# IntptrMax/YoloSharp

Hardware: NVIDIA H100
Metric: images/sec YOLOv8n 3x640x640 (higher is better)
Workload: dtype f16

## Files before the change

yolosharp_b200/csrc/conv_tc.cu:

```cuda
#include <cuda.h>

#include <algorithm>
#include <cstdio>
#include <cstdlib>
#include <cstring>
#include <map>
#include <vector>

#include "common.cuh"
#include "tc_ptx.cuh"

namespace yb {

typedef CUresult (*EncodeTiledFn)(CUtensorMap*, CUtensorMapDataType, cuuint32_t, void*, const cuuint64_t*,
                                  const cuuint64_t*, const cuuint32_t*, const cuuint32_t*, CUtensorMapInterleave,
                                  CUtensorMapSwizzle, CUtensorMapL2promotion, CUtensorMapFloatOOBfill);
static EncodeTiledFn get_encode_fn(std::string* err);

enum TcMode { TC_TAP = 0, TC_HALO = 1, TC_S2P = 2 };

struct TcArgs {
  CUtensorMap tmA;
  const uint8_t* wpk;
  __half* out;
  const __half* res;
  const float* bias;
  int out_pitch, out_coff, res_pitch, res_coff;
  int Ho, Wo;
  int imgs;
  int tiles_w, tiles_h;
  int BW, BH;
  int n_tile, n_tiles;
  int ksz, stride, pad;
  int Cin, BK, chunks;
  int act;
  int mode;
  int stages_a, stages_b;
  uint32_t a_bytes, b_bytes;
  uint32_t a_stride, b_stride;
  uint32_t sbo_a, sbo_b;
  uint32_t row_bytes;
  uint32_t layout_a, layout_b;
  int total_tiles;
  int b_resident;
  int ksteps;
  int epi_mode, dA, dCtot, da0, dch0, dWl, dHW;
  float dstride;
  float* pred;
  uint64_t m_ntiles, m_tpi, m_tw, m_bw;
  int* done_ctr;
  const int* dep_ctr;
  int dep_expect;
  uint64_t m_ohw;
  int* tile_ctr;
  int tile_batch;
  long long* dbg;
  const uint8_t* w2;
  const float* bias2;
  uint32_t w2_off, w2_bytes, b2_stride, sbo_b2, layout_b2;
  int BK2, n2, act1;
};

struct TcConvPlan {
  TcArgs args;
  ConvParams p;
  bool flat;
  int occ;
  bool small;
  size_t smem;
  int grid;
  uint8_t* wpk = nullptr;
  void (*kernel)(TcArgs) = nullptr;
  int fold16 = 0;
};

__device__ __forceinline__ int fdiv(int x, uint64_t magic) { return (int)(((uint64_t)(uint32_t)x * magic) >> 40); }

__device__ __forceinline__ float silu_fast(float v) { return __fdividef(v, 1.0f + __expf(-v)); }
__device__ __forceinline__ float silu_tanh(float v) {
  const float h = 0.5f * v;
  float t;
  asm("tanh.approx.f32 %0, %1;" : "=f"(t) : "f"(h));
  return fmaf(h, t, h);
}

__device__ __forceinline__ uint32_t pack_h2(float x, float y) {
  const __half2 h = __floats2half2_rn(x, y);
  return *reinterpret_cast<const uint32_t*>(&h);
}

constexpr int TC_CONSUMERS = 256;
constexpr int TC_THREADS = TC_CONSUMERS + 32;
constexpr int TC_CONSUMER_WARPS = TC_CONSUMERS / 32;
constexpr int TC_MAX_COUT = 1024;
constexpr int TC_MAX_STAGES = 12;
constexpr int HALO_BW = 8, HALO_BH = 16;

constexpr int TQ = 32;
__device__ __forceinline__ void tq_publish(int* s_tile, volatile int* s_head, int li, int tile) {
  s_tile[li & (TQ - 1)] = tile;
  __threadfence_block();
  *s_head = li + 1;
}
__device__ __forceinline__ int tq_get(const int* s_tile, const volatile int* s_head, int li) {
  const long long t0 = clock64();
  while (*s_head <= li)
    if (clock64() - t0 > 4000000000ll) __trap();
  __threadfence_block();
  return reinterpret_cast<const volatile int*>(s_tile)[li & (TQ - 1)];
}
struct TileDraw {
  int tile, nxt, left, batch, total;
  int* ctr;
  __device__ __forceinline__ TileDraw(int* c, int b, int tot)
      : tile((int)blockIdx.x), nxt(tot), left(1), batch(b), total(tot), ctr(c) {
    if (ctr && tile < total) nxt = (int)gridDim.x + atomicAdd(ctr, batch);
  }
  __device__ __forceinline__ void advance() {
    if (!ctr) { tile += gridDim.x; return; }
    if (--left > 0) { tile++; return; }
    tile = nxt;
    left = batch;
    if (tile < total) nxt = (int)gridDim.x + atomicAdd(ctr, batch);
  }
};

__device__ __forceinline__ void dep_wait_image(const int* ctr, int img, int expect) {
  const long long t0 = clock64();
  while (true) {
    int v;
    asm volatile("ld.acquire.gpu.global.s32 %0, [%1];" : "=r"(v) : "l"(ctr + img) : "memory");
    if (v >= expect) break;
    __nanosleep(100);
    if (clock64() - t0 > 4000000000ll) __trap();
  }
}

template <int NT16, int KK>
__device__ __forceinline__ void tc_mainloop(const TcArgs& a, float* acc, int wg, uint32_t smemA, uint32_t smemB, uint32_t fullA,
                                            uint32_t emptyA, uint32_t fullB, uint32_t emptyB, int& sa, uint32_t& pa, int& sb,
                                            uint32_t& pb) {
  const bool resident = a.b_resident != 0, halo = a.mode != TC_TAP, s2p = a.mode == TC_S2P;
  const uint32_t a_hi = wg_desc_hi(a.sbo_a, a.layout_a), b_hi = wg_desc_hi(a.sbo_b, a.layout_b);
  const uint32_t a_stride16 = a.a_stride >> 4, b_stride16 = a.b_stride >> 4;
  const uint32_t a_lo0 = wg_desc_lo(smemA) + (uint32_t)wg * 8 * a.sbo_a;
  const uint32_t b_lo0 = wg_desc_lo(smemB);
  constexpr uint32_t ROW16 = KK * 2;
  const int ra = a.stages_a, rb = a.stages_b;
  const bool leader = (threadIdx.x & 31) == 0;
  uint32_t pend0 = 0, pend1 = 0;
  uint32_t scale = 0;
  auto step = [&](uint32_t a_lo, uint32_t b_lo, uint32_t relA, uint32_t relB) {
    wg_fence();
#pragma unroll
    for (int k = 0; k < KK; k++) {
      wg_mma_n<NT16, false>(acc, a_lo + 2 * k, a_hi, b_lo + 2 * k, b_hi, ROW16, scale);
      scale = 1;
    }
    wg_commit();
    wg_wait<1>();
    __syncwarp();
    if (leader) {
      if (pend0) mbar_arrive(pend0);
      if (pend1) mbar_arrive(pend1);
    }
    pend0 = relA;
    pend1 = relB;
  };
  if (halo) {
    for (int ch = 0; ch < a.chunks; ch++) {
      mbar_wait(fullA + 8 * sa, pa);
      const uint32_t a_lo = a_lo0 + sa * a_stride16;
      const uint32_t slotA = emptyA + 8 * sa;
      if (++sa == ra) { sa = 0; pa ^= 1; }
#pragma unroll
      for (int t = 0; t < 9; t++) {
        const uint32_t TAP_HALO = (uint32_t)((t / 3) * (HALO_BW + 2) + (t % 3)) * ROW16;
        const uint32_t TAP_S2P = (uint32_t)((t / 3) * (HALO_BW + 1) + (t % 3 != 0 ? 1 : 0)) * 2 * ROW16 +
                                 (t % 3 != 1 ? ROW16 : 0);
// ... 252 lines not shown
      if (a.b_resident)
        for (int ks = 0; ks < a.ksteps; ks++)
          bulk_load_1d(smemB + ks * a.b_stride, a.wpk + (size_t)ks * a.b_stride, a.b_bytes, bfull);
      if (N2_16 > 0) bulk_load_1d(smem0 + a.w2_off, a.w2, a.w2_bytes, bfull);
    }
  }
  if (a.dep_ctr == nullptr) asm volatile("griddepcontrol.wait;" ::: "memory");

  const bool dyn = a.tile_ctr != nullptr;
  if (warp == TC_CONSUMER_WARPS) {
    if (lane == 0) {
      const int ra = a.stages_a, rb = a.b_resident ? 0 : a.stages_b;
      int sa = 0, sb = 0;
      uint32_t pa = 0, pb = 0;
      int li = 0;
      TileDraw td(a.tile_ctr, a.tile_batch, a.total_tiles);
      int dep_ready = -1;
      for (; td.tile < a.total_tiles; li++) {
        const int tile = td.tile;
        if (a.dep_ctr != nullptr) {
          const int mt0 = fdiv(tile, a.m_ntiles);
          int i0, i1;
          if (a.imgs == 1 && a.Ho == 1) {
            const int p0 = mt0 * 128, p1 = min(p0 + 127, a.Wo - 1);
            i0 = fdiv(p0, a.m_ohw); i1 = fdiv(p1, a.m_ohw);
          } else {
            i0 = i1 = fdiv(mt0, a.m_tpi);
          }
          if (i1 != dep_ready || i0 != i1) {
            for (int im = i0; im <= i1; im++)
              if (im != dep_ready) dep_wait_image(a.dep_ctr, im, a.dep_expect);
            dep_ready = i1;
            asm volatile("fence.proxy.async.global;" ::: "memory");
          }
        }
        if (dyn) tq_publish(s_tile, &s_head, li, tile);
        const int mt = fdiv(tile, a.m_ntiles);
        const int nt = tile - mt * a.n_tiles;
        const int img = fdiv(mt, a.m_tpi);
        const int r = mt - img * tiles_per_img;
        const int th = fdiv(r, a.m_tw), tw = r - th * a.tiles_w;
        const int wbase = tw * a.BW * a.stride - a.pad;
        const int hbase = th * a.BH * a.stride - a.pad;
        auto load_b = [&](int t, int ch) {
          mbar_wait(emptyB + 8 * sb, pb ^ 1);
          mbar_arrive_expect_tx(fullB + 8 * sb, a.b_bytes);
          bulk_load_1d(smemB + sb * a.b_stride, a.wpk + (size_t)((nt * taps + t) * a.chunks + ch) * a.b_stride, a.b_bytes,
                       fullB + 8 * sb);
          if (++sb == rb) { sb = 0; pb ^= 1; }
        };
        if (a.mode != TC_TAP) {
          for (int ch = 0; ch < a.chunks; ch++) {
            mbar_wait(emptyA + 8 * sa, pa ^ 1);
            mbar_arrive_expect_tx(fullA + 8 * sa, a.a_bytes);
            tma_load_4d(smemA + sa * a.a_stride, &a.tmA, fullA + 8 * sa, ch * a.BK, a.mode == TC_S2P ? tw * a.BW - 1 : wbase,
                        hbase, img);
            if (++sa == ra) { sa = 0; pa ^= 1; }
            if (!a.b_resident)
              for (int t = 0; t < taps; t++) load_b(t, ch);
          }
        } else {
          for (int t = 0; t < taps; t++) {
            const int kh = a.ksz == 3 ? (t >= 6 ? 2 : (t >= 3 ? 1 : 0)) : 0, kw = t - kh * a.ksz;
            for (int ch = 0; ch < a.chunks; ch++) {
              mbar_wait(emptyA + 8 * sa, pa ^ 1);
              mbar_arrive_expect_tx(fullA + 8 * sa, a.a_bytes);
              tma_load_4d(smemA + sa * a.a_stride, &a.tmA, fullA + 8 * sa, ch * a.BK, wbase + kw, hbase + kh, img);
              if (++sa == ra) { sa = 0; pa ^= 1; }
              if (!a.b_resident) load_b(t, ch);
            }
          }
        }
        td.advance();
      }
      if (dyn) tq_publish(s_tile, &s_head, li, -1);
    }
  } else {
    const int wg = warp >> 2;
    int sa = 0, sb = 0;
    uint32_t pa = 0, pb = 0;
    if (a.b_resident || N2_16 > 0) mbar_wait(bfull, 0);
    int pend_img = -1, pend_cnt = 0;
    const bool dbg_on = a.dbg && blockIdx.x == 0 && threadIdx.x == 0;
    for (int li = 0;; li++) {
      const int tile = dyn ? tq_get(s_tile, &s_head, li) : (int)blockIdx.x + li * (int)gridDim.x;
      if (tile < 0 || tile >= a.total_tiles) break;
      if (dbg_on && li < 16) a.dbg[li * 8 + 0] = clock64();
      float acc[NT16 * 8];
      switch (a.BK) {
        case 64: tc_mainloop<NT16, 4>(a, acc, wg, smemA, smemB, fullA, emptyA, fullB, emptyB, sa, pa, sb, pb); break;
        case 32: tc_mainloop<NT16, 2>(a, acc, wg, smemA, smemB, fullA, emptyA, fullB, emptyB, sa, pa, sb, pb); break;
        default: tc_mainloop<NT16, 1>(a, acc, wg, smemA, smemB, fullA, emptyA, fullB, emptyB, sa, pa, sb, pb); break;
      }
      if (dbg_on && li < 16) a.dbg[li * 8 + 3] = clock64();
      const int mt = fdiv(tile, a.m_ntiles);
      const int nt = tile - mt * a.n_tiles;
      const int img = fdiv(mt, a.m_tpi);
      const int r = mt - img * tiles_per_img;
      const int th = fdiv(r, a.m_tw), tw = r - th * a.tiles_w;
      const int n0 = nt * a.n_tile;
      if constexpr (N2_16 > 0) {
        switch (a.BK2) {
          case 64: tc_fold<NT16, N2_16, 4>(a, acc, s_bias, s_bias + TC_FOLD_BIAS, smem0 + a.w2_off, img, th, tw, wg); break;
          case 32: tc_fold<NT16, N2_16, 2>(a, acc, s_bias, s_bias + TC_FOLD_BIAS, smem0 + a.w2_off, img, th, tw, wg); break;
          default: tc_fold<NT16, N2_16, 1>(a, acc, s_bias, s_bias + TC_FOLD_BIAS, smem0 + a.w2_off, img, th, tw, wg); break;
        }
        if (dbg_on && li < 16) a.dbg[li * 8 + 6] = clock64();
        continue;
      }
      bool valid[2];
      int wo[2];
      tc_epilogue<NT16>(a, acc, s_bias + n0, n0, img, th, tw, wg, valid, wo);
      if (a.done_ctr != nullptr && a.epi_mode == EPI_STORE) {
        const bool flat1 = a.imgs == 1 && a.Ho == 1;
        const int im[2] = {flat1 ? fdiv(min(wo[0], a.Wo - 1), a.m_ohw) : img, flat1 ? fdiv(min(wo[1], a.Wo - 1), a.m_ohw) : img};
        chain_count(a, valid, im, pend_img, pend_cnt);
      }
      if (dbg_on && li < 16) a.dbg[li * 8 + 6] = clock64();
    }
    if (pend_img >= 0) {
      __threadfence();
      __syncwarp();
      if (lane == 0) atomicAdd(a.done_ctr + pend_img, pend_cnt);
    }
  }
}

__global__ void pack_weights_kernel(const __half* __restrict__ w, uint8_t* __restrict__ out, int n_tile, int n_tiles,
                                    int taps, int chunks, int BK, int Cin, uint32_t b_stride, long long pieces) {
  const long long i = (long long)blockIdx.x * blockDim.x + threadIdx.x;
  if (i >= pieces) return;
  const int c16 = BK / 8;
  const int c = (int)(i % c16);
  long long q = i / c16;
  const int r = (int)(q % n_tile); q /= n_tile;
  const int ch = (int)(q % chunks); q /= chunks;
  const int t = (int)(q % taps);
  const int nt = (int)(q / taps);
  const size_t K = (size_t)taps * Cin;
  if (ch * BK + c * 8 >= Cin) return;
  const int4 v = *reinterpret_cast<const int4*>(w + (size_t)(nt * n_tile + r) * K + (size_t)t * Cin + ch * BK + c * 8);
  const int sw = BK == 64 ? (r & 7) : (BK == 32 ? ((r >> 1) & 3) : ((r >> 2) & 1));
  uint8_t* slab = out + (size_t)((nt * taps + t) * chunks + ch) * b_stride;
  *reinterpret_cast<int4*>(slab + (size_t)r * BK * 2 + ((c ^ sw) << 4)) = v;
}

static EncodeTiledFn get_encode_fn(std::string* err) {
  static EncodeTiledFn fn = nullptr;
  if (fn) return fn;
  void* p = nullptr;
  cudaDriverEntryPointQueryResult qres;
  cudaError_t e = cudaGetDriverEntryPoint("cuTensorMapEncodeTiled", &p, cudaEnableDefault, &qres);
  if (e != cudaSuccess || qres != cudaDriverEntryPointSuccess || !p) {
    if (err) *err = "cuTensorMapEncodeTiled entry point not found";
    cudaGetLastError();
    return nullptr;
  }
  fn = (EncodeTiledFn)p;
  return fn;
}

bool tc_conv_supported(const ConvParams& p) {
  if (p.Cin % 16 || p.Cout % 16 || p.Cout > TC_MAX_COUT) return false;
  if (!((p.k == 1 && p.stride == 1) || (p.k == 3 && (p.stride == 1 || p.stride == 2)))) return false;
  if (p.in.coff % 8 || p.in.pitch % 8 || p.out.coff % 8 || p.out.pitch % 8) return false;
  if (p.res.base && (p.res.coff % 8 || p.res.pitch % 8)) return false;
  return true;
}

static int plan_small() {
  const char* v = getenv("YB_PLAN_SMALL");
  return v ? atoi(v) : 0;
}

static int pick_n_tile(int cout) {
  const int cap = plan_small() ? 128 : 256;
  if (cout <= cap) return cout;
  int best = 16;
  for (int n = 16; n <= cap; n += 16)
    if (cout % n == 0) best = n;
  return best;
}

static int tc_num_sms() {
  static int num_sms = 0;
  if (!num_sms) {
    int dev = 0;
    cudaGetDevice(&dev);
    cudaDeviceGetAttribute(&num_sms, cudaDevAttrMultiProcessorCount, dev);
  }
  return num_sms;
}

static bool tc_size_rings(TcConvPlan* plan, size_t extra, int max_occ) {
  TcArgs& a = plan->args;
  const ConvParams& p = plan->p;
  const int num_sms = tc_num_sms();
  const size_t b_all = (size_t)a.ksteps * a.b_stride;
  const int m_tiles = plan->flat ? (p.B * p.Ho * p.Wo + 127) / 128
                                 : p.B * ((p.Wo + a.BW - 1) / a.BW) * ((p.Ho + a.BH - 1) / a.BH);
  const size_t full = 200 * 1024 > extra ? 200 * 1024 - extra : 0;
  plan->occ = 1;
  a.stages_a = 0;
  for (int occ = 2; occ >= 1; occ--) {
    const size_t budget = occ == 2 ? (104 * 1024 > extra ? 104 * 1024 - extra : 0) : full;
    const bool small = m_tiles * a.n_tiles <= 2 * num_sms;
    if (occ == 2 && (a.n_tile > 64 || max_occ < 2)) continue;
    a.b_resident = (a.n_tiles == 1 && b_all + 3 * (size_t)a.a_stride <= budget) ? 1 : 0;
    if (occ == 2 && !plan_small() && !small && !a.b_resident && a.n_tiles == 1 && b_all + 3 * (size_t)a.a_stride <= full) continue;
    if (a.b_resident) {
      a.stages_a = (int)std::min<size_t>(a.mode != TC_TAP ? (a.chunks > 1 ? 8 : 6) : TC_MAX_STAGES, (budget - b_all) / a.a_stride);
      a.stages_b = 0;
    } else if (a.mode != TC_TAP) {
      a.stages_a = (int)std::min<size_t>(3, std::max<size_t>(2, (budget / 3) / a.a_stride));
      const size_t rest = budget > (size_t)a.stages_a * a.a_stride ? budget - (size_t)a.stages_a * a.a_stride : 0;
      a.stages_b = (int)std::min<size_t>(TC_MAX_STAGES, rest / a.b_stride);
    } else {
      a.stages_a = a.stages_b = (int)std::min<size_t>(8, budget / (a.a_stride + a.b_stride));
    }
    const size_t rings = (size_t)a.stages_a * a.a_stride + (a.b_resident ? b_all : (size_t)a.stages_b * a.b_stride);
    a.w2_off = (uint32_t)rings;
    plan->smem = rings + extra + 1024;
    const bool fits = a.stages_a >= 2 && (a.b_resident || a.stages_b >= ((occ == 2 && a.mode != TC_TAP) ? 3 : 2)) && rings <= budget;
    if (fits && (occ == 1 || small || a.stages_a >= 3 || plan_small())) { plan->occ = occ; break; }
    if (occ == 1) a.stages_a = 0;
  }
  plan->small = m_tiles * a.n_tiles <= 2 * num_sms;
  plan->grid = num_sms * plan->occ;
  if (plan_small() && plan->occ == 2) plan->grid = num_sms;
  return !(a.stages_a < 2 || (!a.b_resident && a.stages_b < 2));
}

TcConvPlan* tc_conv_plan_create(const ConvParams& p, std::string* err) {
  EncodeTiledFn encode = get_encode_fn(err);
  if (!encode) return nullptr;
  TcConvPlan* plan = new TcConvPlan();
  plan->p = p;
  TcArgs& a = plan->args;
  memset(&a, 0, sizeof(a));
  a.out = reinterpret_cast<__half*>(p.out.base);
  a.res = reinterpret_cast<const __half*>(p.res.base);
  a.bias = p.bias;
  a.out_pitch = p.out.pitch; a.out_coff = p.out.coff;
  a.res_pitch = p.res.pitch; a.res_coff = p.res.coff;
  a.ksz = p.k; a.stride = p.stride; a.pad = p.pad;
  a.Cin = p.Cin;
  const bool s2p_ok = p.k == 3 && p.stride == 2 && p.in.coff == 0 && p.in.pitch == p.Cin && p.Cin <= 32 && p.in.W % 2 == 0;
  a.mode = (p.k == 3 && p.stride == 1) ? TC_HALO : (s2p_ok ? TC_S2P : TC_TAP);
  auto padded = [&](int bk) { return (p.Cin + bk - 1) / bk * bk; };
  a.BK = padded(64) * 100 <= p.Cin * 135 ? 64 : (padded(32) * 100 <= p.Cin * 135 ? 32 : 16);
  a.chunks = (p.Cin + a.BK - 1) / a.BK;
  a.act = p.act;
  a.n_tile = pick_n_tile(p.Cout);
  a.n_tiles = p.Cout / a.n_tile;
  const CUtensorMapSwizzle swz = a.BK == 64 ? CU_TENSOR_MAP_SWIZZLE_128B
                                            : (a.BK == 32 ? CU_TENSOR_MAP_SWIZZLE_64B : CU_TENSOR_MAP_SWIZZLE_32B);
  a.layout_a = a.layout_b = a.BK == 64 ? 1 : (a.BK == 32 ? 2 : 3);
  a.row_bytes = a.BK * 2;
  a.sbo_a = a.sbo_b = (8 * a.row_bytes) >> 4;
  CUtensorMapSwizzle swz_a = swz;
  if (a.mode == TC_S2P) {
    swz_a = a.BK == 32 ? CU_TENSOR_MAP_SWIZZLE_128B : CU_TENSOR_MAP_SWIZZLE_64B;
    a.layout_a = a.BK == 32 ? 1 : 2;
  }

  plan->flat = (p.k == 1 && p.stride == 1);
  const size_t esz = 2;
  cuuint64_t gdim[4], gstr[3];
  cuuint32_t box[4], estr[4];
  char* base = reinterpret_cast<char*>(p.in.base) + (size_t)p.in.coff * esz;
  if (plan->flat) {
    const cuuint64_t npix = (cuuint64_t)p.B * p.in.H * p.in.W;
    gdim[0] = p.Cin; gdim[1] = npix; gdim[2] = 1; gdim[3] = 1;
    gstr[0] = (cuuint64_t)p.in.pitch * esz; gstr[1] = gstr[0] * npix; gstr[2] = gstr[1];
    a.BW = 128; a.BH = 1;
    box[0] = a.BK; box[1] = 128; box[2] = 1; box[3] = 1;
    estr[0] = estr[1] = estr[2] = estr[3] = 1;
  } else {
    gdim[0] = p.Cin; gdim[1] = p.in.W; gdim[2] = p.in.H; gdim[3] = p.B;
    gstr[0] = (cuuint64_t)p.in.pitch * esz;
    gstr[1] = gstr[0] * p.in.W;
    gstr[2] = gstr[1] * p.in.H;
    if (a.mode == TC_HALO) {
      a.BW = HALO_BW; a.BH = HALO_BH;
      a.sbo_a = ((a.BW + 2) * a.row_bytes) >> 4;
      box[0] = a.BK; box[1] = a.BW + 2; box[2] = a.BH + 2; box[3] = 1;
      estr[0] = estr[1] = estr[2] = estr[3] = 1;
    } else if (a.mode == TC_S2P) {
      a.BW = HALO_BW; a.BH = HALO_BH;
      a.sbo_a = (2 * (a.BW + 1) * 2 * a.row_bytes) >> 4;
      gdim[0] = 2 * p.Cin; gdim[1] = p.in.W / 2;
      gstr[0] = (cuuint64_t)2 * p.in.pitch * esz;
      box[0] = 2 * a.BK; box[1] = a.BW + 1; box[2] = 2 * a.BH + 1; box[3] = 1;
      estr[0] = estr[1] = estr[2] = estr[3] = 1;
    } else {
      double best = -1;
      for (int bw = 1; bw <= std::min(p.Wo, 128); bw++) {
        const int bh = std::min(p.Ho, 128 / bw);
        if (bw * p.stride > 256 || bh * p.stride > 256) continue;
        const double tiles = (double)((p.Wo + bw - 1) / bw) * ((p.Ho + bh - 1) / bh);
        const double eff = (double)p.Wo * p.Ho / (tiles * 128.0);
        if (eff > best + 1e-9 || (eff > best - 1e-9 && bw > a.BW)) { best = eff; a.BW = bw; a.BH = bh; }
      }
      box[0] = a.BK; box[1] = a.BW * p.stride; box[2] = a.BH * p.stride; box[3] = 1;
      estr[0] = 1; estr[1] = p.stride; estr[2] = p.stride; estr[3] = 1;
    }
  }
  CUresult cr = encode(&a.tmA, CU_TENSOR_MAP_DATA_TYPE_FLOAT16, 4, base, gdim, gstr, box, estr,
                       CU_TENSOR_MAP_INTERLEAVE_NONE, swz_a, CU_TENSOR_MAP_L2_PROMOTION_L2_128B,
                       CU_TENSOR_MAP_FLOAT_OOB_FILL_NONE);
  if (cr != CUDA_SUCCESS) {
    if (err) *err = "cuTensorMapEncodeTiled(A) failed with code " + std::to_string((int)cr);
    delete plan;
    return nullptr;
  }
  const int a_rows = a.mode == TC_HALO ? (a.BW + 2) * (a.BH + 2)
                                       : (a.mode == TC_S2P ? 2 * (a.BW + 1) * (2 * a.BH + 1) : a.BW * a.BH);
  a.a_bytes = (uint32_t)(a_rows * a.row_bytes);
  a.b_bytes = (uint32_t)(a.n_tile * a.row_bytes);
  a.a_stride = (uint32_t)((std::max(a_rows, 128) * a.row_bytes + 1023) / 1024 * 1024);
  a.b_stride = (uint32_t)((a.n_tile * a.row_bytes + 1023) / 1024 * 1024);
  a.ksteps = p.k * p.k * a.chunks;
  {
    const size_t total = (size_t)a.n_tiles * a.ksteps * a.b_stride;
    if (cudaMalloc(&plan->wpk, total) != cudaSuccess) {
      if (err) *err = "cudaMalloc(packed weights) failed";
      cudaGetLastError();
      delete plan;
      return nullptr;
    }
    cudaMemset(plan->wpk, 0, total);
    const int chunks16 = a.BK / 8;
    const long long pieces = (long long)a.n_tiles * a.ksteps * a.n_tile * chunks16;
    pack_weights_kernel<<<(unsigned)((pieces + 255) / 256), 256>>>(reinterpret_cast<const __half*>(p.w), plan->wpk, a.n_tile,
                                                                    a.n_tiles, p.k * p.k, a.chunks, a.BK, p.Cin,
                                                                    a.b_stride, pieces);
    if (cudaDeviceSynchronize() != cudaSuccess) {
      if (err) *err = std::string("pack_weights_kernel failed: ") + cudaGetErrorString(cudaGetLastError());
      cudaFree(plan->wpk);
      delete plan;
      return nullptr;
    }
    a.wpk = plan->wpk;
  }
  if (!tc_size_rings(plan, 0, tc_ctas_per_sm(a.n_tile / 16, 0))) {
    if (err) *err = "tile does not fit in shared memory";
    delete plan;
    return nullptr;
  }
  a.epi_mode = p.dec.mode;
  a.dA = p.dec.A; a.dCtot = p.dec.Ctot; a.da0 = p.dec.a0; a.dch0 = p.dec.ch0; a.dWl = p.dec.Wl; a.dHW = p.dec.HW;
  a.dstride = p.dec.stride;
  if (a.epi_mode != EPI_STORE && !(plan->flat && a.n_tiles == 1 && (a.epi_mode != EPI_DFL_BOX || a.n_tile == 64))) {
    if (err) *err = "fused decode epilogue needs a flattened 1x1 conv with a single N tile";
    delete plan;
    return nullptr;
  }
  dispatch_nt16(a.n_tile / 16, [&](auto nt16) { plan->kernel = conv_tc_kernel<decltype(nt16)::value>; });
  {
    cudaFuncSetAttribute(plan->kernel, cudaFuncAttributePreferredSharedMemoryCarveout, cudaSharedmemCarveoutMaxShared);
    cudaError_t ce = cudaFuncSetAttribute(plan->kernel, cudaFuncAttributeMaxDynamicSharedMemorySize, 202 * 1024);
    if (ce != cudaSuccess) {
      if (err) *err = std::string("cudaFuncSetAttribute(conv_tc_kernel) failed: ") + cudaGetErrorString(ce);
      delete plan;
      return nullptr;
    }
  }
  return plan;
}

static void (*tc_fold_kernel(int nt16, int n2_16))(TcArgs) {
#define YB_FOLD_KERNEL(N, N2) \
  if (nt16 == N && n2_16 == N2) return conv_tc_kernel<N, N2>;
  YB_FOLD_KERNEL(2, 2)
  YB_FOLD_KERNEL(4, 4)
  YB_FOLD_KERNEL(5, 4)
  YB_FOLD_KERNEL(5, 5)
  YB_FOLD_KERNEL(8, 5)
  YB_FOLD_KERNEL(8, 8)
#undef YB_FOLD_KERNEL
  return nullptr;
}

TcConvPlan* tc_fold_plan_create(const TcConvPlan* pa, const TcConvPlan* pb, std::string* err) {
  const TcArgs &a1 = pa->args, &a2 = pb->args;
  const ConvParams &p1 = pa->p, &p2 = pb->p;
  auto fail = [&](const std::string& m) -> TcConvPlan* { if (err) *err = m; return nullptr; };
  if (a1.n_tiles != 1) return fail("the producer splits Cout over " + std::to_string(a1.n_tiles) + " N tiles");
  if (a1.epi_mode != EPI_STORE || p1.res.base || (p1.act != ACT_SILU && p1.act != ACT_NONE))
    return fail("the producer is not a plain conv that stores its output");
  if (!pb->flat || a2.n_tiles != 1 || p2.res.base || p2.Cin != p1.Cout || p2.Cout > TC_FOLD_BIAS)
    return fail("the consumer is not a single-tile 1x1 over the producer's channels");
  const int nt16 = a1.n_tile / 16, n2_16 = p2.Cout / 16;
  const int f16 = tc_fold_pass16(n2_16);
  TcConvPlan* plan = new TcConvPlan(*pa);
  plan->wpk = nullptr;
  plan->fold16 = f16;
  TcArgs& a = plan->args;
  a.w2 = a2.wpk; a.bias2 = p2.bias;
  a.w2_bytes = (uint32_t)(a2.ksteps * a2.b_stride);
  a.b2_stride = a2.b_stride; a.sbo_b2 = a2.sbo_b; a.layout_b2 = a2.layout_b;
  a.BK2 = a2.BK; a.n2 = p2.Cout; a.act1 = a1.act;
  a.out = a2.out; a.out_pitch = a2.out_pitch; a.out_coff = a2.out_coff;
  a.res = nullptr; a.res_pitch = a.res_coff = 0;
  a.act = a2.act;
  a.epi_mode = a2.epi_mode;
  a.dA = a2.dA; a.dCtot = a2.dCtot; a.da0 = a2.da0; a.dch0 = a2.dch0; a.dWl = a2.dWl; a.dHW = a2.dHW; a.dstride = a2.dstride;
  if (!tc_size_rings(plan, a.w2_bytes, tc_ctas_per_sm(nt16, n2_16))) {
    delete plan;
    return fail("the producer's rings and the 1x1's " + std::to_string(a.w2_bytes / 1024) + " KiB of weights do not fit in shared memory");
  }
  void (*kernel)(TcArgs) = tc_fold_kernel(nt16, n2_16);
  if (!kernel || (a2.epi_mode == EPI_DFL_BOX && f16 != 4)) {
    delete plan;
    return fail("no fold instantiation for " + std::to_string(a1.n_tile) + " -> " + std::to_string(p2.Cout) + " channels");
  }
  plan->kernel = kernel;
  cudaFuncSetAttribute(kernel, cudaFuncAttributePreferredSharedMemoryCarveout, cudaSharedmemCarveoutMaxShared);
  const cudaError_t ce = cudaFuncSetAttribute(kernel, cudaFuncAttributeMaxDynamicSharedMemorySize, 202 * 1024);
  if (ce != cudaSuccess) {
    delete plan;
    return fail(std::string("cudaFuncSetAttribute(conv_tc_kernel) failed: ") + cudaGetErrorString(ce));
  }
  return plan;
}

std::string tc_conv_plan_describe(const TcConvPlan* plan) {
  const TcArgs& a = plan->args;
  char buf[320];
  int n = snprintf(buf, sizeof(buf), "mode %d BK %d chunks %d n_tile %d x%d stages a/b %d/%d resident %d occ %d threads %d smem %zu KiB grid %d",
                   a.mode, a.BK, a.chunks, a.n_tile, a.n_tiles, a.stages_a, a.stages_b, a.b_resident, plan->occ, TC_THREADS,
                   plan->smem / 1024, plan->grid);
  if (plan->fold16 && n > 0 && n < (int)sizeof(buf))
    snprintf(buf + n, sizeof(buf) - n, " fold 1x1 %d->%d BK %d pass %d w2 %u KiB", a.n_tile, a.n2, a.BK2, 16 * plan->fold16,
             a.w2_bytes / 1024);
  return buf;
}

void tc_conv_plan_destroy(TcConvPlan* plan) {
  if (plan && plan->wpk) cudaFree(plan->wpk);
  delete plan;
}

long long* g_tc_dbg = nullptr;
int g_tc_dbg_countdown = -1;

int tc_conv_rows_per_image(const TcConvPlan* plan) { return plan->p.Ho * plan->p.Wo * plan->args.n_tiles; }

int tc_conv_launch(const TcConvPlan* plan, int B, float* pred, int* tile_ctr, cudaStream_t s, const TcChain* chain) {
  TcArgs a = plan->args;
  a.pred = pred;
  if (chain) {
    a.done_ctr = chain->done_ctr;
    a.dep_ctr = chain->dep_ctr;
    a.dep_expect = chain->dep_expect;
  }
  a.tile_ctr = tile_ctr;
  a.dbg = nullptr;
  if (g_tc_dbg && g_tc_dbg_countdown >= 0 && g_tc_dbg_countdown-- == 0) a.dbg = g_tc_dbg;
  const ConvParams& p = plan->p;
  if (plan->flat) {
    a.imgs = 1;
    a.Ho = 1;
    a.Wo = B * p.Ho * p.Wo;
    a.tiles_h = 1;
    a.tiles_w = (a.Wo + 127) / 128;
  } else {
    a.imgs = B;
    a.Ho = p.Ho; a.Wo = p.Wo;
    a.tiles_w = (p.Wo + a.BW - 1) / a.BW;
    a.tiles_h = (p.Ho + a.BH - 1) / a.BH;
  }
  a.total_tiles = a.imgs * a.tiles_w * a.tiles_h * a.n_tiles;
  auto magic = [](int d) { return (uint64_t)(((((unsigned __int128)1) << 40) + d - 1) / (unsigned)d); };
  a.m_ntiles = magic(a.n_tiles); a.m_tpi = magic(a.tiles_w * a.tiles_h); a.m_tw = magic(a.tiles_w); a.m_bw = magic(a.BW);
  a.m_ohw = magic(p.Ho * p.Wo);
  int grid = std::min(plan->grid, a.total_tiles);
  static const int chain_grid1 = getenv("YB_CHAIN_GRID1") ? atoi(getenv("YB_CHAIN_GRID1")) : 1;
  if (chain && chain_grid1 && plan->occ == 2) grid = std::min(grid, std::max(1, plan->grid / 2));
  if (plan->p.share_sms && a.total_tiles <= 4 * plan->grid && a.ksteps * (a.BK >> 4) <= 40)
    grid = std::max(1, std::min(grid, (a.total_tiles + 2) / 3));
  a.tile_batch = std::max(1, std::min(8, a.total_tiles / (4 * grid)));
  cudaLaunchConfig_t cfg = {};
  cfg.gridDim = dim3(grid);
  cfg.blockDim = dim3(TC_THREADS);
  cfg.dynamicSmemBytes = plan->smem;
  cfg.stream = s;
  cudaLaunchAttribute attr[1];
  attr[0].id = cudaLaunchAttributeProgrammaticStreamSerialization;
  attr[0].val.programmaticStreamSerializationAllowed = 1;
  cfg.attrs = attr;
  static const bool no_pdl = getenv("YB_DEBUG_NO_PDL") != nullptr;
  cfg.numAttrs = no_pdl ? 0 : 1;
  YB_CUDA_CHECK(cudaLaunchKernelEx(&cfg, plan->kernel, a));
  return 0;
}

constexpr int BN_PITCH = HALO_BW + 4;
constexpr int BN_XROWS = BN_PITCH * (HALO_BH + 4);
constexpr int BN_TROWS = BN_PITCH * (HALO_BH + 2);
constexpr int BN_MAX_C = 64;
constexpr size_t BN_MAX_RINGS = 220 * 1024;

struct BnArgs {
  CUtensorMap tmX;
  const uint8_t *w1, *w2;
  const float *bias1, *bias2;
  __half* out;
  int out_pitch, out_coff;
  int shortcut;
  int H, W, tiles_w, tiles_h, total_tiles;
  uint64_t m_tpi, m_tw;
  int cmid, cout;
  int BK1, chunks1, BK2, chunks2;
  uint32_t layout1, layout2;
  uint32_t x_bytes, x_stride, slot;
  uint32_t w1_bytes, w2_bytes, b1_stride, b2_stride;
  uint32_t t_stride;
  int stages;
  int* tile_ctr;
  int tile_batch;
};

struct TcBneckPlan {
  BnArgs args;
  size_t smem;
  int grid, occ;
  void (*kernel)(BnArgs) = nullptr;
};

__device__ __forceinline__ uint32_t sw_off(uint32_t r, uint32_t b, uint32_t rb) {
  const uint32_t sw = rb == 128 ? (r & 7) : (rb == 64 ? ((r >> 1) & 3) : ((r >> 2) & 1));
  return r * rb + ((((b >> 4) ^ sw)) << 4) + (b & 15);
}

template <int NM16, int KK>
__device__ __forceinline__ void bn_stage1(const BnArgs& a, float (&acc)[2][NM16 * 8], uint32_t xslot, uint32_t w1, int wg) {
  constexpr uint32_t RB16 = KK * 2;
  const uint32_t hi = wg_desc_hi(8 * RB16, a.layout1);
  uint32_t scale = 0;
  wg_fence();
  for (int ch = 0; ch < a.chunks1; ch++) {
    const uint32_t a_lo = wg_desc_lo(xslot + ch * a.x_stride) + (uint32_t)wg * 128 * RB16;
#pragma unroll
    for (int t = 0; t < 9; t++) {
      const uint32_t tap = (uint32_t)((t / 3) * BN_PITCH + t % 3) * RB16;
      const uint32_t b_lo = wg_desc_lo(w1 + (t * a.chunks1 + ch) * a.b1_stride);
#pragma unroll
      for (int k = 0; k < KK; k++) {
#pragma unroll
        for (int j = 0; j < 2; j++) wg_mma_n<NM16, false>(acc[j], a_lo + j * 64 * RB16 + tap + 2 * k, hi, b_lo + 2 * k, hi, RB16, scale);
        scale = 1;
      }
    }
  }
  wg_commit();
  wg_wait<0>();
  wg_fence_acc<NM16 * 8>(acc[0]);
  wg_fence_acc<NM16 * 8>(acc[1]);
}

template <int NO16, int KK>
__device__ __forceinline__ void bn_stage2(const BnArgs& a, float* acc, uint32_t tbase, uint32_t w2, int wg) {
  constexpr uint32_t RB16 = KK * 2;
  const uint32_t a_hi = wg_desc_hi(BN_PITCH * RB16, a.layout2), b_hi = wg_desc_hi(8 * RB16, a.layout2);
  uint32_t scale = 0;
  wg_fence();
  for (int ch = 0; ch < a.chunks2; ch++) {
    const uint32_t a_lo = wg_desc_lo(tbase + ch * a.t_stride) + (uint32_t)wg * 8 * BN_PITCH * RB16;
#pragma unroll
    for (int t = 0; t < 9; t++) {
      const uint32_t tap = (uint32_t)((t / 3) * BN_PITCH + t % 3) * RB16;
      const uint32_t b_lo = wg_desc_lo(w2 + (t * a.chunks2 + ch) * a.b2_stride);
#pragma unroll
      for (int k = 0; k < KK; k++) {
        wg_mma_n<NO16, false>(acc, a_lo + tap + 2 * k, a_hi, b_lo + 2 * k, b_hi, RB16, scale);
        scale = 1;
      }
    }
  }
  wg_commit();
  wg_wait<0>();
  wg_fence_acc<NO16 * 8>(acc);
}

__host__ __device__ constexpr int bn_ctas_per_sm(int nm16, int no16) { return nm16 == 1 && no16 <= 2 ? 3 : (nm16 <= 2 && no16 <= 2 ? 2 : 1); }

__device__ __forceinline__ uint32_t ld_shared_u32(uint32_t addr) {
  uint32_t v;
  asm volatile("ld.shared.b32 %0, [%1];" : "=r"(v) : "r"(addr) : "memory");
  return v;
}
__device__ __forceinline__ void st_shared_u32(uint32_t addr, uint32_t v) {
  asm volatile("st.shared.b32 [%0], %1;" ::"r"(addr), "r"(v) : "memory");
}
__device__ __forceinline__ void consumers_sync() { asm volatile("bar.sync 1, %0;" ::"n"(TC_CONSUMERS) : "memory"); }

template <int NM16, int NO16>
__global__ void __launch_bounds__(TC_THREADS, bn_ctas_per_sm(NM16, NO16)) bneck_tc_kernel(const __grid_constant__ BnArgs a) {
  extern __shared__ __align__(1024) uint8_t bn_smem[];
  __shared__ __align__(8) uint64_t bars[2 * TC_MAX_STAGES + 1];
  __shared__ int s_tile[TQ];
  __shared__ volatile int s_head;
  __shared__ __align__(16) float s_bias1[BN_MAX_C], s_bias2[BN_MAX_C];

  const int warp = threadIdx.x >> 5, lane = threadIdx.x & 31;
  for (int i = threadIdx.x; i < a.cmid; i += blockDim.x) s_bias1[i] = a.bias1[i];
  for (int i = threadIdx.x; i < a.cout; i += blockDim.x) s_bias2[i] = a.bias2[i];
  const uint32_t sX = (smem_u32(bn_smem) + 1023u) & ~1023u;
  const uint32_t sW1 = sX + a.stages * a.slot, sW2 = sW1 + a.w1_bytes, sT = sW2 + a.w2_bytes;
  const uint32_t full = smem_u32(&bars[0]), empty = smem_u32(&bars[TC_MAX_STAGES]), wfull = smem_u32(&bars[2 * TC_MAX_STAGES]);
  for (uint32_t i = threadIdx.x; i < a.chunks2 * a.t_stride / 16; i += blockDim.x) st_shared_v4(sT + 16 * i, make_int4(0, 0, 0, 0));
  asm volatile("fence.proxy.async.shared::cta;" ::: "memory");

  asm volatile("griddepcontrol.launch_dependents;" ::: "memory");
  if (warp == TC_CONSUMER_WARPS && lane == 0) {
    s_head = 0;
    for (int s = 0; s < a.stages; s++) {
      mbar_init(full + 8 * s, 1);
      mbar_init(empty + 8 * s, TC_CONSUMER_WARPS);
    }
    mbar_init(wfull, 1);
    asm volatile("fence.mbarrier_init.release.cluster;" ::: "memory");
    asm volatile("fence.proxy.async.shared::cta;" ::: "memory");
  }
  __syncthreads();
  if (warp == TC_CONSUMER_WARPS && lane == 0) {
    asm volatile("prefetch.tensormap [%0];" ::"l"(&a.tmX) : "memory");
    mbar_arrive_expect_tx(wfull, a.w1_bytes + a.w2_bytes);
    bulk_load_1d(sW1, a.w1, a.w1_bytes, wfull);
    bulk_load_1d(sW2, a.w2, a.w2_bytes, wfull);
  }
  asm volatile("griddepcontrol.wait;" ::: "memory");

  const int tiles_per_img = a.tiles_w * a.tiles_h;
  if (warp == TC_CONSUMER_WARPS) {
    if (lane == 0) {
      int s = 0, li = 0;
      uint32_t ph = 0;
      TileDraw td(a.tile_ctr, a.tile_batch, a.total_tiles);
      for (; td.tile < a.total_tiles; li++) {
        const int tile = td.tile;
        tq_publish(s_tile, &s_head, li, tile);
        const int img = fdiv(tile, a.m_tpi), r = tile - img * tiles_per_img;
        const int th = fdiv(r, a.m_tw), tw = r - th * a.tiles_w;
        mbar_wait(empty + 8 * s, ph ^ 1);
        mbar_arrive_expect_tx(full + 8 * s, a.chunks1 * a.x_bytes);
        for (int ch = 0; ch < a.chunks1; ch++)
          tma_load_4d(sX + s * a.slot + ch * a.x_stride, &a.tmX, full + 8 * s, ch * a.BK1, tw * HALO_BW - 2, th * HALO_BH - 2, img);
        if (++s == a.stages) { s = 0; ph ^= 1; }
        td.advance();
      }
      tq_publish(s_tile, &s_head, li, -1);
    }
    return;
  }
  const int wg = warp >> 2, g = lane >> 2, t4 = lane & 3;
  const uint32_t rb1 = a.BK1 * 2, rb2 = a.BK2 * 2;
  int s = 0;
  uint32_t ph = 0;
  mbar_wait(wfull, 0);
  for (int li = 0;; li++) {
    const int tile = tq_get(s_tile, &s_head, li);
    if (tile < 0) break;
    const int img = fdiv(tile, a.m_tpi), r = tile - img * tiles_per_img;
    const int th = fdiv(r, a.m_tw), tw = r - th * a.tiles_w;
    const int h0 = th * HALO_BH, w0 = tw * HALO_BW;
    const uint32_t xslot = sX + s * a.slot;
    mbar_wait(full + 8 * s, ph);
    float acc1[2][NM16 * 8];
    switch (a.BK1) {
      case 64: bn_stage1<NM16, 4>(a, acc1, xslot, sW1, wg); break;
      case 32: bn_stage1<NM16, 2>(a, acc1, xslot, sW1, wg); break;
      default: bn_stage1<NM16, 1>(a, acc1, xslot, sW1, wg); break;
    }
    uint32_t res[2][NO16 * 2];
    if (a.shortcut) {
#pragma unroll
      for (int h = 0; h < 2; h++) {
        const int row = wg * 64 + (warp & 3) * 16 + g + 8 * h;
        const uint32_t xr = (uint32_t)(((row >> 3) + 2) * BN_PITCH + (row & 7) + 2);
#pragma unroll
        for (int J = 0; J < NO16 * 2; J++) {
          const int c = 8 * J + 2 * t4;
          res[h][J] = ld_shared_u32(xslot + (c / a.BK1) * a.x_stride + sw_off(xr, (c % a.BK1) * 2, rb1));
        }
      }
      asm volatile("fence.proxy.async.shared::cta;" ::: "memory");
    }
    __syncwarp();
    if (lane == 0) mbar_arrive(empty + 8 * s);
    if (++s == a.stages) { s = 0; ph ^= 1; }
    consumers_sync();
#pragma unroll
    for (int j = 0; j < 2; j++)
#pragma unroll
      for (int h = 0; h < 2; h++) {
        const int row = (2 * wg + j) * 64 + (warp & 3) * 16 + g + 8 * h;
        const int hh = row / BN_PITCH, ww = row - hh * BN_PITCH;
        if (row >= BN_TROWS || ww >= HALO_BW + 2) continue;
        const int y = h0 - 1 + hh, x = w0 - 1 + ww;
        const bool inside = y >= 0 && y < a.H && x >= 0 && x < a.W;
#pragma unroll
        for (int J = 0; J < NM16 * 2; J++) {
          const int c = 8 * J + 2 * t4;
          float f0 = 0.f, f1 = 0.f;
          if (inside) {
            const float2 b = *reinterpret_cast<const float2*>(s_bias1 + c);
            f0 = silu_tanh(acc1[j][4 * J + 2 * h] + b.x);
            f1 = silu_tanh(acc1[j][4 * J + 2 * h + 1] + b.y);
          }
          const __half2 v = __floats2half2_rn(f0, f1);
          st_shared_u32(sT + (c / a.BK2) * a.t_stride + sw_off((uint32_t)row, (c % a.BK2) * 2, rb2),
                        *reinterpret_cast<const uint32_t*>(&v));
        }
      }
    asm volatile("fence.proxy.async.shared::cta;" ::: "memory");
    consumers_sync();
    float acc2[NO16 * 8];
    switch (a.BK2) {
      case 64: bn_stage2<NO16, 4>(a, acc2, sT, sW2, wg); break;
      case 32: bn_stage2<NO16, 2>(a, acc2, sT, sW2, wg); break;
      default: bn_stage2<NO16, 1>(a, acc2, sT, sW2, wg); break;
    }
#pragma unroll
    for (int h = 0; h < 2; h++) {
      const int row = wg * 64 + (warp & 3) * 16 + g + 8 * h;
      const int y = h0 + (row >> 3), x = w0 + (row & 7);
      if (y >= a.H || x >= a.W) continue;
      __half* orow = a.out + ((size_t)(img * a.H + y) * a.W + x) * a.out_pitch + a.out_coff;
#pragma unroll
      for (int J = 0; J < NO16 * 2; J++) {
        const int c = 8 * J + 2 * t4;
        const float2 b = *reinterpret_cast<const float2*>(s_bias2 + c);
        float f0 = silu_tanh(acc2[4 * J + 2 * h] + b.x), f1 = silu_tanh(acc2[4 * J + 2 * h + 1] + b.y);
        if (a.shortcut) {
          const float2 xv = __half22float2(*reinterpret_cast<const __half2*>(&res[h][J]));
          f0 += xv.x; f1 += xv.y;
        }
        *reinterpret_cast<__half2*>(orow + c) = __floats2half2_rn(f0, f1);
      }
    }
  }
}

TcBneckPlan* tc_bneck_plan_create(const TcConvPlan* pa, const TcConvPlan* pb, std::string* err) {
  const ConvParams &p1 = pa->p, &p2 = pb->p;
  const TcArgs &a1 = pa->args, &a2 = pb->args;
  auto fail = [&](const char* m) -> TcBneckPlan* { if (err) *err = m; return nullptr; };
  if (a1.mode != TC_HALO || a2.mode != TC_HALO || a1.n_tiles != 1 || a2.n_tiles != 1 || p1.Cout != p2.Cin ||
      p1.Cout > BN_MAX_C || p2.Cout > BN_MAX_C || p1.act != ACT_SILU || p2.act != ACT_SILU || p1.res.base ||
      a1.epi_mode != EPI_STORE || a2.epi_mode != EPI_STORE)
    return fail("not a fusable 3x3 / 3x3 pair");
  const bool shortcut = p2.res.base != nullptr;
  if (shortcut && (p2.res.base != p1.in.base || p2.res.coff != p1.in.coff || p2.res.pitch != p1.in.pitch || p1.Cin != p2.Cout))
    return fail("shortcut is not the block input");
  EncodeTiledFn encode = get_encode_fn(err);
  if (!encode) return nullptr;
  TcBneckPlan* plan = new TcBneckPlan();
  BnArgs& a = plan->args;
  memset(&a, 0, sizeof(a));
  const size_t esz = 2;
  cuuint64_t gdim[4] = {(cuuint64_t)p1.Cin, (cuuint64_t)p1.in.W, (cuuint64_t)p1.in.H, (cuuint64_t)p1.B};
  cuuint64_t gstr[3];
  gstr[0] = (cuuint64_t)p1.in.pitch * esz;
  gstr[1] = gstr[0] * p1.in.W;
  gstr[2] = gstr[1] * p1.in.H;
  cuuint32_t box[4] = {(cuuint32_t)a1.BK, (cuuint32_t)BN_PITCH, (cuuint32_t)(HALO_BH + 4), 1}, estr[4] = {1, 1, 1, 1};
  const CUtensorMapSwizzle swz = a1.BK == 64 ? CU_TENSOR_MAP_SWIZZLE_128B : (a1.BK == 32 ? CU_TENSOR_MAP_SWIZZLE_64B : CU_TENSOR_MAP_SWIZZLE_32B);
  CUresult cr = encode(&a.tmX, CU_TENSOR_MAP_DATA_TYPE_FLOAT16, 4, reinterpret_cast<char*>(p1.in.base) + (size_t)p1.in.coff * esz,
                       gdim, gstr, box, estr, CU_TENSOR_MAP_INTERLEAVE_NONE, swz, CU_TENSOR_MAP_L2_PROMOTION_L2_128B,
                       CU_TENSOR_MAP_FLOAT_OOB_FILL_NONE);
  if (cr != CUDA_SUCCESS) {
    delete plan;
    return fail("cuTensorMapEncodeTiled(bottleneck input) failed");
  }
  a.w1 = a1.wpk; a.w2 = a2.wpk;
  a.bias1 = p1.bias; a.bias2 = p2.bias;
  a.out = reinterpret_cast<__half*>(p2.out.base);
  a.out_pitch = p2.out.pitch; a.out_coff = p2.out.coff;
  a.shortcut = shortcut;
  a.H = p2.Ho; a.W = p2.Wo;
  a.cmid = p1.Cout; a.cout = p2.Cout;
  a.BK1 = a1.BK; a.chunks1 = a1.chunks; a.layout1 = a1.layout_a;
  a.BK2 = a2.BK; a.chunks2 = a2.chunks; a.layout2 = a2.layout_a;
  auto kib = [](size_t b) { return (uint32_t)((b + 1023) / 1024 * 1024); };
  a.x_bytes = (uint32_t)(BN_XROWS * a.BK1 * 2);
  a.x_stride = kib(a.x_bytes);
  a.slot = a.chunks1 * a.x_stride;
  a.b1_stride = a1.b_stride; a.b2_stride = a2.b_stride;
  a.w1_bytes = (uint32_t)(a1.ksteps * a1.b_stride);
  a.w2_bytes = (uint32_t)(a2.ksteps * a2.b_stride);
  a.t_stride = kib((size_t)BN_TROWS * a.BK2 * 2);
  const size_t fixed = (size_t)a.w1_bytes + a.w2_bytes + (size_t)a.chunks2 * a.t_stride;
  const int nm16 = a.cmid / 16, no16 = a.cout / 16;
  plan->occ = 0;
  for (int occ = bn_ctas_per_sm(nm16, no16); occ >= 1 && !plan->occ; occ--) {
    const size_t budget = occ == 3 ? 72 * 1024 : (occ == 2 ? 104 * 1024 : BN_MAX_RINGS);
    if (fixed >= budget) continue;
    a.stages = (int)std::min<size_t>(4, (budget - fixed) / a.slot);
    if (a.stages >= occ) plan->occ = occ;
  }
  if (!plan->occ) {
    delete plan;
    return fail("bottleneck tile does not fit in shared memory");
  }
  if (plan->occ == 1 && !shortcut) {
    delete plan;
    return fail("one CTA per SM and no shortcut: the unfused pair is as fast");
  }
  plan->smem = (size_t)a.stages * a.slot + fixed + 1024;
  dispatch_nt16(nm16, [&](auto m) {
    dispatch_nt16(no16, [&](auto o) {
      constexpr int M = decltype(m)::value, O = decltype(o)::value;
      if constexpr (M <= BN_MAX_C / 16 && O <= BN_MAX_C / 16) plan->kernel = bneck_tc_kernel<M, O>;
    });
  });
  cudaFuncSetAttribute(plan->kernel, cudaFuncAttributePreferredSharedMemoryCarveout, cudaSharedmemCarveoutMaxShared);
  static std::map<void (*)(BnArgs), size_t> smem_limit;
  size_t& lim = smem_limit[plan->kernel];
  if (plan->smem > lim) {
    cudaError_t ce = cudaFuncSetAttribute(plan->kernel, cudaFuncAttributeMaxDynamicSharedMemorySize, (int)plan->smem);
    if (ce != cudaSuccess) {
      delete plan;
      return fail("cudaFuncSetAttribute(bneck_tc_kernel) failed");
    }
    lim = plan->smem;
  }
  int dev = 0, num_sms = 0;
  cudaGetDevice(&dev);
  cudaDeviceGetAttribute(&num_sms, cudaDevAttrMultiProcessorCount, dev);
  plan->grid = num_sms * plan->occ;
  return plan;
}

std::string tc_bneck_plan_describe(const TcBneckPlan* plan) {
  const BnArgs& a = plan->args;
  char buf[256];
  snprintf(buf, sizeof(buf), "fused bottleneck %d->%d BK %d/%d chunks %d/%d shortcut %d stages %d occ %d smem %zu KiB grid %d",
           a.cmid, a.cout, a.BK1, a.BK2, a.chunks1, a.chunks2, a.shortcut, a.stages, plan->occ, plan->smem / 1024, plan->grid);
  return buf;
}

void tc_bneck_plan_destroy(TcBneckPlan* plan) { delete plan; }

int tc_bneck_launch(const TcBneckPlan* plan, int B, int* tile_ctr, cudaStream_t s) {
  BnArgs a = plan->args;
  a.tiles_w = (a.W + HALO_BW - 1) / HALO_BW;
  a.tiles_h = (a.H + HALO_BH - 1) / HALO_BH;
  a.total_tiles = B * a.tiles_w * a.tiles_h;
  auto magic = [](int d) { return (uint64_t)(((((unsigned __int128)1) << 40) + d - 1) / (unsigned)d); };
  a.m_tpi = magic(a.tiles_w * a.tiles_h); a.m_tw = magic(a.tiles_w);
  a.tile_ctr = tile_ctr;
  const int grid = std::min(plan->grid, a.total_tiles);
  a.tile_batch = std::max(1, std::min(8, a.total_tiles / (4 * grid)));
  cudaLaunchConfig_t cfg = {};
  cfg.gridDim = dim3(grid);
  cfg.blockDim = dim3(TC_THREADS);
  cfg.dynamicSmemBytes = plan->smem;
  cfg.stream = s;
  cudaLaunchAttribute attr[1];
  attr[0].id = cudaLaunchAttributeProgrammaticStreamSerialization;
  attr[0].val.programmaticStreamSerializationAllowed = 1;
  cfg.attrs = attr;
  cfg.numAttrs = 1;
  YB_CUDA_CHECK(cudaLaunchKernelEx(&cfg, plan->kernel, a));
  return 0;
}

constexpr int ST_TW = 16, ST_TH = 8;
constexpr int ST_THREADS = 128;

struct StemArgs {
  const void* in;
  const __half* w16;
  const float* bias;
  __half* out;
  int out_pitch, out_coff;
  int B, H, W, Ho, Wo, Cout;
  int src_H, src_W;
  uint32_t pad_h2;
  int tiles_w, tiles_h, total_tiles;
  uint64_t m_tpi, m_tw;
};

template <int DT>
__device__ __forceinline__ uint2 stem_load4(const void* in, size_t rowbase, int col, bool lo_ok) {
  uint2 r = make_uint2(0u, 0u);
  if (DT == YB_F16) {
    const uint32_t* p = reinterpret_cast<const uint32_t*>(reinterpret_cast<const __half*>(in) + rowbase + col);
    if (lo_ok) r.x = __ldg(p);
    r.y = __ldg(p + 1);
  } else if (DT == YB_U8) {
    const uint16_t* p = reinterpret_cast<const uint16_t*>(reinterpret_cast<const uint8_t*>(in) + rowbase + col);
    const __half2 k2 = __float2half2_rn(1.0f / 255.0f);
    const __half2 c2 = __hmul2(k2, __float2half2_rn(-1024.0f));
    auto cvt = [&](uint32_t v) {
      const uint32_t x = __byte_perm(v, 0x64006400u, 0x7150);
      const __half2 h = __hfma2(*reinterpret_cast<const __half2*>(&x), k2, c2);
      return *reinterpret_cast<const uint32_t*>(&h);
    };
    if (lo_ok) r.x = cvt(__ldg(p));
    r.y = cvt(__ldg(p + 1));
  } else {
    const float2* p = reinterpret_cast<const float2*>(reinterpret_cast<const float*>(in) + rowbase + col);
    if (lo_ok) { const float2 v = __ldg(p); r.x = pack_h2(v.x, v.y); }
    const float2 v = __ldg(p + 1);
    r.y = pack_h2(v.x, v.y);
  }
  return r;
}

template <int DT>
__device__ __forceinline__ uint32_t stem_load1(const void* in, size_t i) {
  if (DT == YB_F16) return (uint32_t)__ldg(reinterpret_cast<const unsigned short*>(in) + i);
  if (DT == YB_U8) {
    const __half k = __float2half_rn(1.0f / 255.0f);
    const uint32_t x = 0x6400u | (uint32_t)__ldg(reinterpret_cast<const uint8_t*>(in) + i);
    const unsigned short xs = (unsigned short)x;
    const __half h = __hfma(*reinterpret_cast<const __half*>(&xs), k, __hmul(k, __float2half_rn(-1024.0f)));
    return (uint32_t)*reinterpret_cast<const unsigned short*>(&h);
  }
  const __half h = __float2half_rn(__ldg(reinterpret_cast<const float*>(in) + i));
  return (uint32_t)*reinterpret_cast<const unsigned short*>(&h);
}

template <int DT>
__device__ __forceinline__ uint2 stem_load4_ragged(const void* in, size_t rowbase, int col, int src_W, uint32_t pad1) {
  uint32_t e[4];
#pragma unroll
  for (int j = 0; j < 4; j++) {
    const int c = col + j;
    e[j] = c < 0 ? 0u : (c >= src_W ? pad1 : stem_load1<DT>(in, rowbase + c));
  }
  return make_uint2(e[0] | (e[1] << 16), e[2] | (e[3] << 16));
}
// ... 153 lines not shown
```

Baseline: 17270.

## Add ping-pong named barriers so consumer warpgroups overlap mainloop with epilogue

Adds a per-plan pingpong flag that makes the two consumer warpgroups take turns running the MMA mainloop, using named barriers, so one warpgroup's epilogue overlaps the other's tensor-core work. It is enabled only for store epilogues where the A and B rings are deep enough to hold a whole tile's k-steps, and can be turned off with YB_NO_EPI_OVERLAP. The change also adds debug clock probes to the fused bottleneck kernel. The cost is serialized mainloops and barrier overhead, which can leave tensor cores idle when the epilogue is short.

```diff
diff --git a/yolosharp_b200/csrc/conv_tc.cu b/yolosharp_b200/csrc/conv_tc.cu
--- a/yolosharp_b200/csrc/conv_tc.cu
+++ b/yolosharp_b200/csrc/conv_tc.cu
@@ -59,6 +59,7 @@
   const float* bias2;
   uint32_t w2_off, w2_bytes, b2_stride, sbo_b2, layout_b2;
   int BK2, n2, act1;
+  int pingpong;
 };
 
 struct TcConvPlan {
@@ -95,6 +96,10 @@
 constexpr int TC_MAX_COUT = 1024;
 constexpr int TC_MAX_STAGES = 12;
 constexpr int HALO_BW = 8, HALO_BH = 16;
+constexpr int TC_BAR_MMA = 2;
+
+__device__ __forceinline__ void named_bar_sync(int id, int n) { asm volatile("bar.sync %0, %1;" ::"r"(id), "r"(n) : "memory"); }
+__device__ __forceinline__ void named_bar_arrive(int id, int n) { asm volatile("bar.arrive %0, %1;" ::"r"(id), "r"(n) : "memory"); }
 
 constexpr int TQ = 32;
 __device__ __forceinline__ void tq_publish(int* s_tile, volatile int* s_head, int li, int tile) {
@@ -513,16 +518,20 @@
     if (a.b_resident || N2_16 > 0) mbar_wait(bfull, 0);
     int pend_img = -1, pend_cnt = 0;
     const bool dbg_on = a.dbg && blockIdx.x == 0 && threadIdx.x == 0;
-    for (int li = 0;; li++) {
+    const bool pp = a.pingpong != 0;
+    int li = 0;
+    for (;; li++) {
       const int tile = dyn ? tq_get(s_tile, &s_head, li) : (int)blockIdx.x + li * (int)gridDim.x;
       if (tile < 0 || tile >= a.total_tiles) break;
       if (dbg_on && li < 16) a.dbg[li * 8 + 0] = clock64();
+      if (pp && (wg == 1 || li > 0)) named_bar_sync(TC_BAR_MMA + wg, TC_CONSUMERS);
       float acc[NT16 * 8];
       switch (a.BK) {
         case 64: tc_mainloop<NT16, 4>(a, acc, wg, smemA, smemB, fullA, emptyA, fullB, emptyB, sa, pa, sb, pb); break;
         case 32: tc_mainloop<NT16, 2>(a, acc, wg, smemA, smemB, fullA, emptyA, fullB, emptyB, sa, pa, sb, pb); break;
         default: tc_mainloop<NT16, 1>(a, acc, wg, smemA, smemB, fullA, emptyA, fullB, emptyB, sa, pa, sb, pb); break;
       }
+      if (pp) named_bar_arrive(TC_BAR_MMA + (wg ^ 1), TC_CONSUMERS);
       if (dbg_on && li < 16) a.dbg[li * 8 + 3] = clock64();
       const int mt = fdiv(tile, a.m_ntiles);
       const int nt = tile - mt * a.n_tiles;
@@ -549,6 +558,7 @@
       }
       if (dbg_on && li < 16) a.dbg[li * 8 + 6] = clock64();
     }
+    if (pp && wg == 0 && li > 0) named_bar_sync(TC_BAR_MMA, TC_CONSUMERS);
     if (pend_img >= 0) {
       __threadfence();
       __syncwarp();
@@ -660,6 +670,14 @@
   plan->grid = num_sms * plan->occ;
   if (plan_small() && plan->occ == 2) plan->grid = num_sms;
   return !(a.stages_a < 2 || (!a.b_resident && a.stages_b < 2));
+}
+
+static int tc_pingpong_fits(const TcConvPlan* plan) {
+  const TcArgs& a = plan->args;
+  const char* off = getenv("YB_NO_EPI_OVERLAP");
+  if (off && atoi(off)) return 0;
+  const int na = a.mode != TC_TAP ? a.chunks : a.ksteps;
+  return a.epi_mode == EPI_STORE && na <= a.stages_a && (a.b_resident || a.ksteps <= a.stages_b) ? 1 : 0;
 }
 
 TcConvPlan* tc_conv_plan_create(const ConvParams& p, std::string* err) {
@@ -780,6 +798,7 @@
     return nullptr;
   }
   a.epi_mode = p.dec.mode;
+  a.pingpong = tc_pingpong_fits(plan);
   a.dA = p.dec.A; a.dCtot = p.dec.Ctot; a.da0 = p.dec.a0; a.dch0 = p.dec.ch0; a.dWl = p.dec.Wl; a.dHW = p.dec.HW;
   a.dstride = p.dec.stride;
   if (a.epi_mode != EPI_STORE && !(plan->flat && a.n_tiles == 1 && (a.epi_mode != EPI_DFL_BOX || a.n_tile == 64))) {
@@ -841,6 +860,7 @@
     delete plan;
     return fail("the producer's rings and the 1x1's " + std::to_string(a.w2_bytes / 1024) + " KiB of weights do not fit in shared memory");
   }
+  a.pingpong = tc_pingpong_fits(plan);
   void (*kernel)(TcArgs) = tc_fold_kernel(nt16, n2_16);
   if (!kernel || (a2.epi_mode == EPI_DFL_BOX && f16 != 4)) {
     delete plan;
@@ -859,9 +879,9 @@
 std::string tc_conv_plan_describe(const TcConvPlan* plan) {
   const TcArgs& a = plan->args;
   char buf[320];
-  int n = snprintf(buf, sizeof(buf), "mode %d BK %d chunks %d n_tile %d x%d stages a/b %d/%d resident %d occ %d threads %d smem %zu KiB grid %d",
+  int n = snprintf(buf, sizeof(buf), "mode %d BK %d chunks %d n_tile %d x%d stages a/b %d/%d resident %d occ %d threads %d smem %zu KiB grid %d pingpong %d",
                    a.mode, a.BK, a.chunks, a.n_tile, a.n_tiles, a.stages_a, a.stages_b, a.b_resident, plan->occ, TC_THREADS,
-                   plan->smem / 1024, plan->grid);
+                   plan->smem / 1024, plan->grid, a.pingpong);
   if (plan->fold16 && n > 0 && n < (int)sizeof(buf))
     snprintf(buf + n, sizeof(buf) - n, " fold 1x1 %d->%d BK %d pass %d w2 %u KiB", a.n_tile, a.n2, a.BK2, 16 * plan->fold16,
              a.w2_bytes / 1024);
@@ -951,6 +971,7 @@
   int stages;
   int* tile_ctr;
   int tile_batch;
+  long long* dbg;
 };
 
 struct TcBneckPlan {
@@ -1091,6 +1112,7 @@
   int s = 0;
   uint32_t ph = 0;
   mbar_wait(wfull, 0);
+  const bool dbg_on = a.dbg && blockIdx.x == 0 && threadIdx.x == 0;
   for (int li = 0;; li++) {
     const int tile = tq_get(s_tile, &s_head, li);
     if (tile < 0) break;
@@ -1098,6 +1120,7 @@
     const int th = fdiv(r, a.m_tw), tw = r - th * a.tiles_w;
     const int h0 = th * HALO_BH, w0 = tw * HALO_BW;
     const uint32_t xslot = sX + s * a.slot;
+    if (dbg_on && li < 16) a.dbg[li * 8 + 0] = clock64();
     mbar_wait(full + 8 * s, ph);
     float acc1[2][NM16 * 8];
     switch (a.BK1) {
@@ -1105,6 +1128,7 @@
       case 32: bn_stage1<NM16, 2>(a, acc1, xslot, sW1, wg); break;
       default: bn_stage1<NM16, 1>(a, acc1, xslot, sW1, wg); break;
     }
+    if (dbg_on && li < 16) a.dbg[li * 8 + 3] = clock64();
     uint32_t res[2][NO16 * 2];
     if (a.shortcut) {
 #pragma unroll
@@ -1154,6 +1178,7 @@
       case 32: bn_stage2<NO16, 2>(a, acc2, sT, sW2, wg); break;
       default: bn_stage2<NO16, 1>(a, acc2, sT, sW2, wg); break;
     }
+    if (dbg_on && li < 16) a.dbg[li * 8 + 4] = clock64();
 #pragma unroll
     for (int h = 0; h < 2; h++) {
       const int row = wg * 64 + (warp & 3) * 16 + g + 8 * h;
@@ -1172,6 +1197,7 @@
         *reinterpret_cast<__half2*>(orow + c) = __floats2half2_rn(f0, f1);
       }
     }
+    if (dbg_on && li < 16) a.dbg[li * 8 + 6] = clock64();
   }
 }
 
@@ -1283,6 +1309,8 @@
   auto magic = [](int d) { return (uint64_t)(((((unsigned __int128)1) << 40) + d - 1) / (unsigned)d); };
   a.m_tpi = magic(a.tiles_w * a.tiles_h); a.m_tw = magic(a.tiles_w);
   a.tile_ctr = tile_ctr;
+  a.dbg = nullptr;
+  if (g_tc_dbg && g_tc_dbg_countdown >= 0 && g_tc_dbg_countdown-- == 0) a.dbg = g_tc_dbg;
   const int grid = std::min(plan->grid, a.total_tiles);
   a.tile_batch = std::max(1, std::min(8, a.total_tiles / (4 * grid)));
   cudaLaunchConfig_t cfg = {};
```

After: 17300, median of 6. About the same (+0.2%).
